# linto-ai/whisper-timestamped

Measured on NVIDIA H100. Metric: audio-sec/s (RTF) large-v3 1h synthetic @1/2/4/8 H100; DTW GB/s vs HBM peak, higher is better.
Workload: dtype bf16x3 tensor-core GEMMs (float32-accurate), f32 elsewhere, f64 DTW accumulate

## Files before the change

whisper-timestamped_b200/csrc/decode_steps.cu:

```cuda
#include "decode_common.cuh"

namespace wts {

constexpr int MG_THREADS = 256;
constexpr int MG_WARPS = MG_THREADS / 32;
constexpr int MG_MAXROWS = 32;
constexpr int MG_MAXNI = 10;

struct MgShared {
    int list[MG_MAXROWS];
    int n_active;
};

__device__ __forceinline__ float4 ldcg4(const float* p) { return __ldcg(reinterpret_cast<const float4*>(p)); }
__device__ __forceinline__ void prefetch_l2(const void* p) { asm volatile("prefetch.global.L2 [%0];" ::"l"(p)); }

enum { EPI_STORE = 0, EPI_ADD = 1, EPI_GELU = 2 };

__device__ __noinline__ void self_attention_task(const WtsDecodeSteps& P, const WtsDecLayer& Lr, int row, int h, int pos,
                                                    float* sc)
{
    const int lane = threadIdx.x & 31;
    const int D = P.D, n_ctx = P.n_ctx;
    float* Kc = Lr.self_k + ((int64_t)row * P.H + h) * n_ctx * 64;
    float* Vc = Lr.self_v + ((int64_t)row * P.H + h) * n_ctx * 64;
    const float* qrow = P.qkv + (int64_t)row * 3 * D + h * 64;
    {
        const float2 kn = __ldcg(reinterpret_cast<const float2*>(qrow + D) + lane);
        const float2 vn = __ldcg(reinterpret_cast<const float2*>(qrow + 2 * D) + lane);
        reinterpret_cast<float2*>(Kc + (int64_t)pos * 64)[lane] = kn;
        reinterpret_cast<float2*>(Vc + (int64_t)pos * 64)[lane] = vn;
        __threadfence_block();
        __syncwarp();
    }
    float q[64];
#pragma unroll
    for (int c = 0; c < 16; ++c) {
        const float4 t = ldcg4(qrow + 4 * c);
        q[4 * c] = t.x; q[4 * c + 1] = t.y; q[4 * c + 2] = t.z; q[4 * c + 3] = t.w;
    }
    const int nk = pos + 1;
    float mx = -CUDART_INF_F;
#pragma unroll 1
    for (int j = lane; j < nk; j += 32) {
        const float* kr = Kc + (int64_t)j * 64;
        float a = 0.f;
#pragma unroll
        for (int c = 0; c < 16; ++c) {
            const float4 kv = ldcg4(kr + 4 * c);
            a += q[4 * c] * kv.x + q[4 * c + 1] * kv.y + q[4 * c + 2] * kv.z + q[4 * c + 3] * kv.w;
        }
        sc[j] = a;
        mx = fmaxf(mx, a);
    }
    mx = warp_max(mx);
    float sum = 0.f;
#pragma unroll 1
    for (int j = lane; j < nk; j += 32) {
        const float e = expf(sc[j] - mx);
        sc[j] = e;
        sum += e;
    }
    sum = warp_sum(sum);
    __syncwarp();
    float2 o = make_float2(0.f, 0.f);
#pragma unroll 8
    for (int j = 0; j < nk; ++j) {
        const float p = sc[j];
        const float2 v = __ldcg(reinterpret_cast<const float2*>(Vc + (int64_t)j * 64) + lane);
        o.x = fmaf(p, v.x, o.x);
        o.y = fmaf(p, v.y, o.y);
    }
    const float inv = 1.0f / sum;
    reinterpret_cast<float2*>(P.att + (int64_t)row * D + h * 64)[lane] = make_float2(o.x * inv, o.y * inv);
    __syncwarp();
}

__device__ __noinline__ void cross_attention_phase(const WtsDecodeSteps& P, const WtsDecLayer& Lr, const MgShared& sh, float* xs)
{
    const int D = P.D, H = P.H;
    CaScratch& sc = *reinterpret_cast<CaScratch*>(xs);
    const int c8 = threadIdx.x & 7;
    for (int t = blockIdx.x; t < sh.n_active * H; t += gridDim.x) {
        const int row = sh.list[t / H], h = t % H;
        float qf[8];
        {
            const float* qp = P.q + (int64_t)row * D + h * 64 + c8 * 8;
            const float4 a = ldcg4(qp), b = ldcg4(qp + 4);
            qf[0] = a.x; qf[1] = a.y; qf[2] = a.z; qf[3] = a.w; qf[4] = b.x; qf[5] = b.y; qf[6] = b.z; qf[7] = b.w;
// ... 29 lines not shown
        }
        if (threadIdx.x == 0) sh.n_active = count <= MG_MAXROWS ? count : 0;
    }
    __syncthreads();
}

__global__ void __launch_bounds__(MG_THREADS)
lean_embed_kernel(const WtsDecodeSteps P)
{
    pdl_launch();
    pdl_wait();
    const int row = blockIdx.x;
    if (row >= P.cap || __ldcg(P.done + row) != 0) return;
    const int nt = __ldcg(P.n_tokens + row);
    const int tok = __ldcg(P.tokens + (int64_t)row * P.cfg.tokens_ld + nt - 1);
    const float* e = P.emb + (int64_t)tok * P.D;
    const float* p = P.pos + (int64_t)(nt - 1) * P.D;
    for (int c = threadIdx.x; c < P.D; c += MG_THREADS) P.x[(int64_t)row * P.D + c] = __ldg(e + c) + __ldg(p + c);
}

__global__ void __launch_bounds__(MG_THREADS)
lean_self_attn_kernel(const WtsDecodeSteps P, const WtsDecLayer* Lr)
{
    extern __shared__ __align__(16) unsigned char smem_raw[];
    MgShared& sh = *reinterpret_cast<MgShared*>(smem_raw);
    float* xs = reinterpret_cast<float*>(smem_raw + 1024);
    pdl_launch();
    pdl_wait();
    build_row_list(P, sh);
    const int warp = threadIdx.x >> 5;
    const int t = blockIdx.x * MG_WARPS + warp;
    if (t >= sh.n_active * P.H) return;
    const int row = sh.list[t / P.H];
    self_attention_task(P, *Lr, row, t % P.H, __ldcg(P.n_tokens + row) - 1, xs + warp * P.n_ctx);
}

__global__ void __launch_bounds__(MG_THREADS)
lean_cross_attn_kernel(const WtsDecodeSteps P, const WtsDecLayer* Lr)
{
    extern __shared__ __align__(16) unsigned char smem_raw[];
    MgShared& sh = *reinterpret_cast<MgShared*>(smem_raw);
    float* xs = reinterpret_cast<float*>(smem_raw + 1024);
    pdl_launch();
    pdl_wait();
    build_row_list(P, sh);
    if (blockIdx.x >= sh.n_active * P.H) return;
    cross_attention_phase(P, *Lr, sh, xs);
}

constexpr int LEAN_SELECT_THREADS = 1024;
__global__ void __launch_bounds__(LEAN_SELECT_THREADS)
lean_select_kernel(const WtsDecodeSteps P)
{
    __shared__ SelectScratch S;
    pdl_launch();
    pdl_wait();
    const int row = blockIdx.x;
    if (row >= P.cap || P.done[row] != 0) return;
    select_row(P.logits + (int64_t)row * P.cfg.n_vocab, P.cfg, P.suppress, P.blank, P.tokens + (int64_t)row * P.cfg.tokens_ld,
               P.n_tokens + row, P.n_prompt[row], P.done + row, P.logprobs + (int64_t)row * P.lp_ld,
               P.full != nullptr ? P.full + (int64_t)row * P.lp_ld * P.cfg.n_vocab : nullptr,
               P.last_full != nullptr ? P.last_full + (int64_t)row * P.cfg.n_vocab : nullptr, S);
}

__device__ __forceinline__ void mma_m16n8k16_bf16(float (&d)[4], uint32_t a0, uint32_t a1, uint32_t a2, uint32_t a3, uint32_t b0,
                                                  uint32_t b1)
{
    asm volatile("mma.sync.aligned.m16n8k16.row.col.f32.bf16.bf16.f32 {%0, %1, %2, %3}, {%4, %5, %6, %7}, {%8, %9}, {%0, %1, %2, %3};"
                 : "+f"(d[0]), "+f"(d[1]), "+f"(d[2]), "+f"(d[3]) : "r"(a0), "r"(a1), "r"(a2), "r"(a3), "r"(b0), "r"(b1));
}
__device__ __forceinline__ uint4 ldg_stream_u4(const void* p)
{
    uint4 v;
    asm volatile("ld.global.nc.L1::no_allocate.v4.u32 {%0, %1, %2, %3}, [%4];" : "=r"(v.x), "=r"(v.y), "=r"(v.z), "=r"(v.w) : "l"(p));
    return v;
}
__device__ __forceinline__ uint32_t pack_bf16x2(float lo_k, float hi_k)
{
    const __nv_bfloat162 v = __floats2bfloat162_rn(lo_k, hi_k);
    return *reinterpret_cast<const uint32_t*>(&v);
}

constexpr int MM_TASK_N = 8;

template <bool LN>
__device__ __forceinline__ void mma_stage(const float* src, int64_t ld, int col0, int kc, const float* __restrict__ gam,
                                          const float* __restrict__ bet, const MgShared& sh, uint32_t* Ah, uint32_t* Al, int pitchW)
{
    const int warp = threadIdx.x >> 5, lane = threadIdx.x & 31;
    const int NI = kc >> 7;
    for (int i = warp; i < sh.n_active; i += MG_WARPS) {
        const float* r = src + (int64_t)sh.list[i] * ld + col0;
        float4 v[MG_MAXNI];
#pragma unroll
        for (int k = 0; k < MG_MAXNI; ++k)
            if (k < NI) v[k] = ldcg4(r + 4 * (lane + 32 * k));
        if (LN) {
            float s = 0.f;
#pragma unroll
            for (int k = 0; k < MG_MAXNI; ++k)
                if (k < NI) s += (v[k].x + v[k].y) + (v[k].z + v[k].w);
            const float mean = warp_sum(s) / (float)kc;
            float q = 0.f;
#pragma unroll
            for (int k = 0; k < MG_MAXNI; ++k)
                if (k < NI) {
                    const float a = v[k].x - mean, b = v[k].y - mean, c = v[k].z - mean, d = v[k].w - mean;
                    q += (a * a + b * b) + (c * c + d * d);
                }
            const float rstd = 1.0f / sqrtf(warp_sum(q) / (float)kc + 1e-5f);
#pragma unroll
            for (int k = 0; k < MG_MAXNI; ++k)
                if (k < NI) {
                    const float4 g = __ldg(reinterpret_cast<const float4*>(gam) + lane + 32 * k);
                    const float4 b = __ldg(reinterpret_cast<const float4*>(bet) + lane + 32 * k);
                    v[k].x = (v[k].x - mean) * rstd * g.x + b.x;
                    v[k].y = (v[k].y - mean) * rstd * g.y + b.y;
                    v[k].z = (v[k].z - mean) * rstd * g.z + b.z;
                    v[k].w = (v[k].w - mean) * rstd * g.w + b.w;
                }
        }
#pragma unroll
        for (int k = 0; k < MG_MAXNI; ++k)
            if (k < NI) {
                const int f = lane + 32 * k;
                const int kb = f >> 3, j = f & 7;
                const int w0 = kb * 16 + ((j & 1) * 2) * 4 + (j >> 1);
                const float hx = __bfloat162float(__float2bfloat16_rn(v[k].x)), hy = __bfloat162float(__float2bfloat16_rn(v[k].y));
                const float hz = __bfloat162float(__float2bfloat16_rn(v[k].z)), hw = __bfloat162float(__float2bfloat16_rn(v[k].w));
                uint32_t* ah = Ah + (int64_t)i * pitchW;
                uint32_t* al = Al + (int64_t)i * pitchW;
                ah[w0] = pack_bf16x2(hx, hy);
                ah[w0 + 4] = pack_bf16x2(hz, hw);
                al[w0] = pack_bf16x2(v[k].x - hx, v[k].y - hy);
                al[w0 + 4] = pack_bf16x2(v[k].z - hz, v[k].w - hw);
            }
    }
}

template <int MT>
__global__ void __launch_bounds__(MG_THREADS, 1)
lean_mma_kernel(const WtsDecodeSteps P, const __nv_bfloat16* __restrict__ Whi, int64_t plane, int N, int K,
                const float* __restrict__ bias, const float* src, int64_t lds, const float* gam, const float* bet, float* out,
                int64_t ldo, int epi, int ln)
{
    extern __shared__ __align__(16) unsigned char smem_raw[];
    MgShared& sh = *reinterpret_cast<MgShared*>(smem_raw);
    const int D = P.D;
    const int KC = D;
    const int nchunks = K / KC;
    const int pitchW = (KC + 8) >> 1;
    uint32_t* Ah = reinterpret_cast<uint32_t*>(smem_raw + 1024);
    uint32_t* Al = Ah + (size_t)16 * MT * pitchW;
    float4* red = reinterpret_cast<float4*>(Al + (size_t)16 * MT * pitchW);
    const int warp = threadIdx.x >> 5, lane = threadIdx.x & 31;
    const int g = lane >> 2, q = lane & 3;
    const int ntasks = (N + MM_TASK_N - 1) / MM_TASK_N;
    pdl_launch();
    {
        const int lines_per_row = K / 64;
        for (int t = blockIdx.x, r = 0; t < ntasks && r < 2; t += gridDim.x, ++r)
            for (int ln_ = threadIdx.x; ln_ < MM_TASK_N * lines_per_row * 2; ln_ += MG_THREADS) {
                const int pl = ln_ / (MM_TASK_N * lines_per_row), rem = ln_ - pl * MM_TASK_N * lines_per_row;
                const int f = rem / lines_per_row, c = rem - f * lines_per_row;
                prefetch_l2(Whi + (int64_t)pl * plane + (int64_t)min(t * MM_TASK_N + f, N - 1) * K + c * 64);
            }
    }
    pdl_wait();
    build_row_list(P, sh);
    const int nA = sh.n_active;
    if (nA == 0) return;
    for (int idx = threadIdx.x; idx < (16 * MT - nA) * pitchW; idx += MG_THREADS) {
        Ah[(size_t)nA * pitchW + idx] = 0u;
        Al[(size_t)nA * pitchW + idx] = 0u;
    }
    const int nkb = KC >> 5;
    float acc[2][MT][4];
#pragma unroll
    for (int r = 0; r < 2; ++r)
#pragma unroll
        for (int m = 0; m < MT; ++m)
#pragma unroll
            for (int e = 0; e < 4; ++e) acc[r][m][e] = 0.f;

    auto task_partial = [&](int t, int c, float (&part)[MT][4]) {
        const int n = min(t * MM_TASK_N + g, N - 1);
        const __nv_bfloat16* wrow = Whi + (int64_t)n * K + (int64_t)c * KC + 8 * q;
#pragma unroll 1
        for (int kb0 = warp; kb0 < nkb; kb0 += 5 * MG_WARPS) {
            uint4 bh[5], bl[5];
#pragma unroll
            for (int u = 0; u < 5; ++u) {
                const int kb = kb0 + u * MG_WARPS;
                if (kb < nkb) {
                    bh[u] = ldg_stream_u4(wrow + kb * 32);
                    bl[u] = ldg_stream_u4(wrow + kb * 32 + plane);
                }
            }
#pragma unroll
            for (int u = 0; u < 5; ++u) {
                const int kb = kb0 + u * MG_WARPS;
                if (kb < nkb) {
#pragma unroll
                    for (int m = 0; m < MT; ++m) {
                        const uint32_t* ah0 = Ah + (size_t)(16 * m + g) * pitchW + kb * 16 + q;
                        const uint32_t* ah8 = ah0 + (size_t)8 * pitchW;
                        const uint32_t* al0 = Al + (size_t)(16 * m + g) * pitchW + kb * 16 + q;
                        const uint32_t* al8 = al0 + (size_t)8 * pitchW;
                        {
                            const uint32_t a0 = ah0[0], a1 = ah8[0], a2 = ah0[4], a3 = ah8[4];
                            const uint32_t l0 = al0[0], l1 = al8[0], l2 = al0[4], l3 = al8[4];
                            mma_m16n8k16_bf16(part[m], a0, a1, a2, a3, bh[u].x, bh[u].y);
                            mma_m16n8k16_bf16(part[m], l0, l1, l2, l3, bh[u].x, bh[u].y);
                            mma_m16n8k16_bf16(part[m], a0, a1, a2, a3, bl[u].x, bl[u].y);
                        }
                        {
                            const uint32_t a0 = ah0[8], a1 = ah8[8], a2 = ah0[12], a3 = ah8[12];
                            const uint32_t l0 = al0[8], l1 = al8[8], l2 = al0[12], l3 = al8[12];
                            mma_m16n8k16_bf16(part[m], a0, a1, a2, a3, bh[u].z, bh[u].w);
                            mma_m16n8k16_bf16(part[m], l0, l1, l2, l3, bh[u].z, bh[u].w);
                            mma_m16n8k16_bf16(part[m], a0, a1, a2, a3, bl[u].z, bl[u].w);
                        }
                    }
                }
            }
        }
    };
    auto task_finish = [&](int t, float (&part)[MT][4]) {
#pragma unroll
        for (int m = 0; m < MT; ++m) red[(warp * MT + m) * 32 + lane] = make_float4(part[m][0], part[m][1], part[m][2], part[m][3]);
        __syncthreads();
        if (warp < MT) {
            float4 s = red[(0 * MT + warp) * 32 + lane];
#pragma unroll
            for (int w = 1; w < MG_WARPS; ++w) {
                const float4 v = red[(w * MT + warp) * 32 + lane];
                s.x += v.x; s.y += v.y; s.z += v.z; s.w += v.w;
            }
            const float vals[4] = {s.x, s.y, s.z, s.w};
#pragma unroll
            for (int e = 0; e < 4; ++e) {
                const int ri = 16 * warp + g + ((e >> 1) ? 8 : 0);
                const int n = t * MM_TASK_N + 2 * q + (e & 1);
                if (ri < nA && n < N) {
                    float v = vals[e] + (bias != nullptr ? __ldg(bias + n) : 0.f);
                    float* dst = out + (int64_t)sh.list[ri] * ldo + n;
                    if (epi == EPI_GELU) v = gelu_erf(v);
                    else if (epi == EPI_ADD) v += __ldcg(dst);
                    *dst = v;
                }
            }
        }
        __syncthreads();
    };

    for (int c = 0; c < nchunks; ++c) {
        if (c > 0) __syncthreads();
        if (ln) mma_stage<true>(src, lds, c * KC, KC, gam, bet, sh, Ah, Al, pitchW);
        else    mma_stage<false>(src, lds, c * KC, KC, nullptr, nullptr, sh, Ah, Al, pitchW);
        __syncthreads();
        if (nchunks == 1) {
            for (int t = blockIdx.x; t < ntasks; t += gridDim.x) {
                float part[MT][4];
#pragma unroll
                for (int m = 0; m < MT; ++m)
#pragma unroll
                    for (int e = 0; e < 4; ++e) part[m][e] = 0.f;
                task_partial(t, 0, part);
                task_finish(t, part);
            }
        } else {
#pragma unroll
            for (int r = 0; r < 2; ++r) {
                const int t = blockIdx.x + r * gridDim.x;
                if (t < ntasks) task_partial(t, c, acc[r]);
            }
        }
    }
    if (nchunks > 1) {
#pragma unroll
        for (int r = 0; r < 2; ++r) {
            const int t = blockIdx.x + r * gridDim.x;
            if (t < ntasks) task_finish(t, acc[r]);
        }
    }
}

template <int MT>
static int launch_lean_step(const WtsDecodeSteps& P, const WtsDecLayer* h_layers, int n_sm, cudaStream_t st)
{
    const int D = P.D, H = P.H, V = P.cfg.n_vocab;
    const int pitchW = (D + 8) >> 1;
    const size_t sm_mma = 1024 + (size_t)2 * 16 * MT * pitchW * 4 + (size_t)MG_WARPS * MT * 32 * 16;
    const size_t sm_self = (size_t)MG_WARPS * P.n_ctx * sizeof(float) + 1024;
    const size_t sm_cross = sizeof(CaScratch) + 1024;
    static bool attr = false;
    if (!attr) {
        WTS_CUDA_CHECK(cudaFuncSetAttribute(lean_mma_kernel<MT>, cudaFuncAttributeMaxDynamicSharedMemorySize, 200 * 1024));
        attr = true;
    }
    if (sm_mma > 200 * 1024) { set_error("wts_decode_step_kernels: %zu bytes of shared memory needed", sm_mma); return -2; }
    const dim3 g_gemv(n_sm), blk(MG_THREADS);
    const dim3 g_self((P.max_rows * H + MG_WARPS - 1) / MG_WARPS), g_cross(P.max_rows * H);
    typedef const __nv_bfloat16* BF;
    const float* nof = nullptr;
    WTS_CUDA_CHECK(launch_pdl(lean_embed_kernel, dim3(P.cap), blk, 0, st, P));
    for (int li = 0; li < P.n_layer; ++li) {
        const WtsDecLayer& L = h_layers[li];
        const WtsDecLayer* dL = P.layers + li;
        WTS_CUDA_CHECK(launch_pdl(lean_mma_kernel<MT>, g_gemv, blk, sm_mma, st, P, (BF)L.sb_qkv, (int64_t)L.pl_qkv, 3 * D, D, L.b_qkv,
                                  (const float*)P.x, (int64_t)D, L.ln1_g, L.ln1_b, P.qkv, (int64_t)(3 * D), (int)EPI_STORE, 1));
        WTS_CUDA_CHECK(launch_pdl(lean_self_attn_kernel, g_self, blk, sm_self, st, P, dL));
        WTS_CUDA_CHECK(launch_pdl(lean_mma_kernel<MT>, g_gemv, blk, sm_mma, st, P, (BF)L.sb_o, (int64_t)L.pl_o, D, D, L.b_o,
                                  (const float*)P.att, (int64_t)D, nof, nof, P.x, (int64_t)D, (int)EPI_ADD, 0));
        WTS_CUDA_CHECK(launch_pdl(lean_mma_kernel<MT>, g_gemv, blk, sm_mma, st, P, (BF)L.sb_cq, (int64_t)L.pl_cq, D, D, L.b_cq,
                                  (const float*)P.x, (int64_t)D, L.ln2_g, L.ln2_b, P.q, (int64_t)D, (int)EPI_STORE, 1));
        WTS_CUDA_CHECK(launch_pdl(lean_cross_attn_kernel, g_cross, blk, sm_cross, st, P, dL));
        WTS_CUDA_CHECK(launch_pdl(lean_mma_kernel<MT>, g_gemv, blk, sm_mma, st, P, (BF)L.sb_co, (int64_t)L.pl_co, D, D, L.b_co,
                                  (const float*)P.att, (int64_t)D, nof, nof, P.x, (int64_t)D, (int)EPI_ADD, 0));
        WTS_CUDA_CHECK(launch_pdl(lean_mma_kernel<MT>, g_gemv, blk, sm_mma, st, P, (BF)L.sb_fc1, (int64_t)L.pl_fc1, 4 * D, D, L.b_fc1,
                                  (const float*)P.x, (int64_t)D, L.ln3_g, L.ln3_b, P.mid, (int64_t)(4 * D), (int)EPI_GELU, 1));
        WTS_CUDA_CHECK(launch_pdl(lean_mma_kernel<MT>, g_gemv, blk, sm_mma, st, P, (BF)L.sb_fc2, (int64_t)L.pl_fc2, D, 4 * D, L.b_fc2,
                                  (const float*)P.mid, (int64_t)(4 * D), nof, nof, P.x, (int64_t)D, (int)EPI_ADD, 0));
    }
    WTS_CUDA_CHECK(launch_pdl(lean_mma_kernel<MT>, g_gemv, blk, sm_mma, st, P, (BF)P.emb_sb, (int64_t)P.emb_plane, V, D, nof,
                              (const float*)P.x, (int64_t)D, P.ln_g, P.ln_b, P.logits, (int64_t)V, (int)EPI_STORE, 1));
    WTS_CUDA_CHECK(launch_pdl(lean_select_kernel, dim3(P.cap), dim3(LEAN_SELECT_THREADS), 0, st, P));
    return 0;
}

}

using namespace wts;

extern "C" int wts_decode_step_kernels(const WtsDecodeSteps* p, const WtsDecLayer* h_layers, void* stream)
{
    if (!p || !h_layers) { set_error("wts_decode_step_kernels: null argument"); return -2; }
    const WtsDecodeSteps& P = *p;
    if (P.D % 128 != 0 || P.D > 128 * MG_MAXNI || P.D != P.H * 64) {
        set_error("wts_decode_step_kernels: n_text_state %d not supported", P.D);
        return -2;
    }
    if (P.max_rows > MG_MAXROWS || P.max_rows < 1) { set_error("wts_decode_step_kernels: 1..%d active rows", MG_MAXROWS); return -2; }
    if ((size_t)MG_WARPS * P.n_ctx * sizeof(float) + 1024 > 48 * 1024) { set_error("wts_decode_step_kernels: n_text_ctx too large"); return -2; }
    if (P.emb_sb == nullptr) { set_error("wts_decode_step_kernels: no SB16 token embedding"); return -2; }
    static int n_sm = 0;
    if (n_sm == 0) {
        int dev = 0;
        WTS_CUDA_CHECK(cudaGetDevice(&dev));
        WTS_CUDA_CHECK(cudaDeviceGetAttribute(&n_sm, cudaDevAttrMultiProcessorCount, dev));
    }
    if (P.D / MM_TASK_N > 2 * n_sm) {
        set_error("wts_decode_step_kernels: n_text_state %d needs at least %d SMs, the device has %d", P.D, P.D / 16, n_sm);
        return -2;
    }
    cudaStream_t st = (cudaStream_t)stream;
    return P.max_rows <= 16 ? launch_lean_step<1>(P, h_layers, n_sm, st) : launch_lean_step<2>(P, h_layers, n_sm, st);
}
```

whisper-timestamped_b200/whisper_timestamped/engine.py:

```python
import ctypes
import os

import numpy as np
import torch

from . import _native as nat
from .alignment import attn_prep, dtw, plan_segments, split_jumps
from .model import SB16
from .windows import N_FRAMES, WindowRecord

N_SAMPLES = 480000
N_CTX_AUDIO = 1500
KPAD = 1504


def _i32(x, dev):
    return torch.as_tensor(np.asarray(x, dtype=np.int32)).to(dev)


class CudaEngine:
    def __init__(self, model, max_batch=None, gemm_backend=None, keep_full_logprobs=False, small_batch_rows=None):
        self.m = model
        self.dev = model.device
        self.w = model.w
        self.dims = model.dims
        self.max_batch = max_batch or int(os.environ.get("WTS_MAX_BATCH", "64"))
        self.backend = int(os.environ.get("WTS_GEMM_BACKEND", "0")) if gemm_backend is None else gemm_backend
        self.conv_backend = int(os.environ.get("WTS_CONV_BACKEND", str(self.backend)))
        self.fused_attention = os.environ.get("WTS_FUSED_ATTN", "1") != "0"
        self.keep_full_logprobs = keep_full_logprobs
        self.qk_buffers = []
        self.window_index = []
        self.full_logprobs = []
        self.launches = 0
        self.use_graph = os.environ.get("WTS_CUDA_GRAPH", "1") != "0"
        self.small_batch_rows = min(32, int(os.environ.get("WTS_SMALL_BATCH_ROWS", "8")) if small_batch_rows is None
                                    else int(small_batch_rows))
        self.small_batch_steps = 0
        self.decode_steps_run = 0
        self._graphs = {}
        self.profile = False
        self._events = []
        self.heads = None
        self.set_alignment_heads(model.heads)

    def set_alignment_heads(self, heads=None):
        heads = sorted((int(l), int(h)) for l, h in (self.m.heads if heads is None else heads))
        if heads == self.heads:
            return
        d = self.dims
        L, H = d.n_text_layer, d.n_text_head
        assert heads and all(0 <= l < L and 0 <= h < H for l, h in heads), heads
        assert len(set(heads)) == len(heads), "duplicate alignment heads"
        slots = torch.full((L, H), -1, dtype=torch.int32)
        for s_, (l, h) in enumerate(heads):
            slots[l, h] = s_
        self.heads = heads
        self.head_slot = slots.to(self.dev)
        counts = [sum(1 for l, _ in heads if l == li) for li in range(L)]
        self.layer_slots = [(sum(counts[:li]), counts[li]) for li in range(L)]
        self._session = None
        self._tf_state = None

    class _Phase:
        def __init__(self, eng, name):
            self.eng, self.name = eng, name

        def __enter__(self):
            if self.eng.profile:
                self.a = torch.cuda.Event(enable_timing=True)
                self.b = torch.cuda.Event(enable_timing=True)
                self.a.record(torch.cuda.current_stream(self.eng.dev))

        def __exit__(self, *exc):
            if self.eng.profile:
                self.b.record(torch.cuda.current_stream(self.eng.dev))
                self.eng._events.append((self.name, self.a, self.b))

    def phase(self, name):
        return CudaEngine._Phase(self, name)

    def stage_ms(self, reset=True):
        torch.cuda.synchronize(self.dev)
        out = {}
        self.batch_ms = [(B, steps, self._events[i][1].elapsed_time(self._events[i][2]))
                         for (B, steps, i) in getattr(self, "batch_log", [])]
        self.batch_log = []
        for name, a, b in self._events:
            out[name] = out.get(name, 0.0) + a.elapsed_time(b)
        if reset:
            self._events = []
        return out

    def _st(self):
        return nat.stream_ptr(self.dev)

    def gemm(self, a, b, M, N, K, *, lda=None, ldb=None, a_plane=None, b_plane=None, a_off=0, b_off=0,
             batch=(1, 1), a_b=(0, 0), b_b=(0, 0), alpha=1.0, bias=None, bias_on_m=False, act=0,
             residual=None, ldr=0, r_b=(0, 0), out_f32=None, ldc=0, c_b=(0, 0), c_off=0,
             out_sb=None, ldo=0, o_plane=0, o_b=(0, 0), o_off=0, head_dim=0, head_stride=0,
             a_f32=False, b_f32=False, backend=None, row_mask=None):
        g = nat.Gemm()
        if a_f32:
            g.a, g.lda, g.a_plane = a.data_ptr() + 4 * a_off, lda, 0
        else:
            g.a, g.lda, g.a_plane = a.ptr + 2 * a_off, lda or a.ld, a_plane if a_plane is not None else a.plane
        if b_f32:
            g.b, g.ldb, g.b_plane = b.data_ptr() + 4 * b_off, ldb, 0
        else:
            g.b, g.ldb, g.b_plane = b.ptr + 2 * b_off, ldb or b.ld, b_plane if b_plane is not None else b.plane
        g.a_bo, g.a_bi = a_b
        g.b_bo, g.b_bi = b_b
        g.M, g.N, g.K = M, N, K
        g.batch_outer, g.batch_inner = batch
        g.alpha = alpha
        g.bias = bias.data_ptr() if bias is not None else None
        g.bias_on_m = 1 if bias_on_m else 0
        g.act = act
        if residual is not None:
            g.residual, g.ldr = residual.data_ptr(), ldr
            g.r_bo, g.r_bi = r_b
        if out_f32 is not None:
            g.out_f32, g.ldc = out_f32.data_ptr() + 4 * c_off, ldc
            g.c_bo, g.c_bi = c_b
# ... 203 lines not shown
        limit = self.batch_limit(setup)
        for i in range(0, len(jobs), limit):
            out.extend(self._decode_batch(jobs[i:i + limit], setup))
        return out

    def window_bytes(self, sample_len):
        d = self.dims
        L, H, D, n_ctx = d.n_text_layer, d.n_text_head, d.n_text_state, d.n_text_ctx
        N, ctx = len(self.heads), N_CTX_AUDIO
        cross = L * H * ctx * 64 * 2 * 2 + N * ctx * 64 * 4 + H * ctx * 64 * 4
        self_kv = 2 * L * H * n_ctx * 64 * 4
        rows = 2 * N * (sample_len + 1) * ctx * 4
        Da = d.n_audio_state
        encoder = 3002 * d.n_mels * 4 + 3001 * Da * 4 + ctx * Da * (4 + 4 + 8 + 4 + 16 + 4) + Da * KPAD * 4
        return cross + self_kv + rows + encoder

    def batch_limit(self, setup):
        key = (tuple(self.heads), setup.sample_len)
        lim = getattr(self, "_limits", {})
        if key not in lim:
            torch.cuda.empty_cache()
            free, _ = torch.cuda.mem_get_info(self.dev)
            ses = getattr(self, "_session", None)
            if ses is not None:
                free += ses["cap"] * self.window_bytes(setup.sample_len)
            lim[key] = max(1, min(self.max_batch, int(0.85 * free) // self.window_bytes(setup.sample_len)))
            self._limits = lim
        return lim[key]

    def _decoder_session(self, setup, need):
        d, dev = self.dims, self.dev
        tok = setup.tokenizer
        V, D, n_ctx = d.n_vocab, d.n_text_state, d.n_text_ctx
        ses = getattr(self, "_session", None)
        cap = 4
        while cap < need:
            cap *= 2
        cap = min(cap, max(self.batch_limit(setup), need))
        if ses is not None and ses["cap"] >= need:
            cap = ses["cap"]
        key = (cap, setup.sample_len, tok.eot, tok.timestamp_begin, tok.no_timestamps, setup.max_initial_timestamp_index,
               self.keep_full_logprobs, self.small_batch_rows)
        if ses is not None and ses["key"] == key:
            return ses
        self._session = ses = None
        qk_rows = setup.sample_len + 1
        n_slots = len(self.heads)
        i32 = dict(dtype=torch.int32, device=dev)
        ses = dict(key=key, cap=cap, qk_rows=qk_rows, graph=None, per_step=0)
        ses["st8"] = self._alloc_decoder_state(cap, cap)
        ses["st8"]["hs_fin"] = SB16(cap, D, dev)
        ses["tokens"] = torch.zeros((cap, n_ctx + 1), **i32)
        ses["n_tokens"] = torch.ones(cap, **i32)
        ses["n_prompt"] = torch.ones(cap, **i32)
        ses["done"] = torch.ones(cap, **i32)
        ses["logprobs"] = torch.zeros((cap, qk_rows), dtype=torch.float32, device=dev)
        ses["full"] = torch.empty((cap, qk_rows, V), dtype=torch.float32, device=dev) if self.keep_full_logprobs else None
        ses["qk_buf"] = torch.zeros((cap, max(1, n_slots), qk_rows, N_CTX_AUDIO), dtype=torch.float32, device=dev)
        ses["qk_out"] = torch.zeros_like(ses["qk_buf"])
        ses["qk_out_idx"] = None
        ses["s_tok"] = torch.zeros(cap, **i32)
        ses["s_pos"] = torch.zeros(cap, **i32)
        ses["s_qkr"] = torch.zeros(cap, **i32)
        ses["s_act"] = torch.zeros(cap, **i32)
        ses["seq_ids"] = _i32(list(range(cap)), dev)
        ses["logits"] = torch.empty((cap, V), dtype=torch.float32, device=dev)
        ses["xs"] = torch.empty((cap, D), dtype=torch.float32, device=dev)
        ses["last_full"] = torch.zeros((cap, V), dtype=torch.float32, device=dev)
        ses["suppress"] = torch.zeros(V, dtype=torch.uint8, device=dev)
        ses["blank"] = torch.zeros(V, dtype=torch.uint8, device=dev)
        ses["cfg"] = nat.DecodeCfg(n_vocab=V, eot=tok.eot, timestamp_begin=tok.timestamp_begin,
                                   no_timestamps=tok.no_timestamps,
                                   max_initial_ts=-1 if setup.max_initial_timestamp_index is None else setup.max_initial_timestamp_index,
                                   sample_len=setup.sample_len, n_ctx=n_ctx, tokens_ld=n_ctx + 1)
        ses["steps"] = self._steps_descriptor(ses) if self.small_batch_rows > 0 else None
        self._session = ses
        return ses

    def _steps_descriptor(self, ses):
        d, w, dev = self.dims, self.w, self.dev
        D, H, L, V = d.n_text_state, d.n_text_head, d.n_text_layer, d.n_vocab
        if D % 128 != 0 or D > 1280 or D != 64 * H:
            return None
        if D // 8 > 2 * torch.cuda.get_device_properties(dev).multi_processor_count:
            return None
        st8, cap = ses["st8"], ses["cap"]
        layers = (nat.DecLayer * L)()
        for li, blk in enumerate(w.dec):
            a, c, y = blk.attn, blk.cross, layers[li]
            y.ln1_g, y.ln1_b, y.b_qkv, y.b_o = a.ln_g.data_ptr(), a.ln_b.data_ptr(), a.qkv_b.data_ptr(), a.out_b.data_ptr()
            y.ln2_g, y.ln2_b, y.b_cq, y.b_co = c.ln_g.data_ptr(), c.ln_b.data_ptr(), c.q_b.data_ptr(), c.out_b.data_ptr()
            y.ln3_g, y.ln3_b = blk.mlp_ln_g.data_ptr(), blk.mlp_ln_b.data_ptr()
            y.b_fc1, y.b_fc2 = blk.fc1_b.data_ptr(), blk.fc2_b.data_ptr()
            y.self_k, y.self_v = st8["sk"][li].data_ptr(), st8["sv"][li].data_ptr()
            y.cross_k16, y.cross_v16 = st8["ck"][li].data_ptr(), st8["cv"][li].data_ptr()
            kal = st8["ckal"][li]
            y.cross_k_align, y.head_slot = kal.data_ptr() if kal is not None else None, self.head_slot[li].data_ptr()
            y.align_s0, y.align_n = self.layer_slots[li]
            for name, sb in (("qkv", a.qkv), ("o", a.out), ("cq", c.q), ("co", c.out), ("fc1", blk.fc1), ("fc2", blk.fc2)):
                assert sb.ld == sb.cols
                setattr(y, "sb_" + name, sb.ptr)
                setattr(y, "pl_" + name, sb.plane)
        raw = np.frombuffer(bytes(layers), dtype=np.uint8).copy()
        f32 = dict(dtype=torch.float32, device=dev)
        keep = dict(layers=torch.from_numpy(raw).to(dev), x=torch.zeros((cap, D), **f32), qkv=torch.zeros((cap, 3 * D), **f32),
                    att=torch.zeros((cap, D), **f32), q=torch.zeros((cap, D), **f32), mid=torch.zeros((cap, 4 * D), **f32))
        p = nat.DecodeSteps()
        p.layers = keep["layers"].data_ptr()
        p.emb, p.pos, p.ln_g, p.ln_b = w.emb.data_ptr(), w.dec_pos.data_ptr(), w.ln_g.data_ptr(), w.ln_b.data_ptr()
        p.tokens, p.n_tokens, p.n_prompt, p.done = (ses[k].data_ptr() for k in ("tokens", "n_tokens", "n_prompt", "done"))
        p.logprobs, p.qk_buf = ses["logprobs"].data_ptr(), ses["qk_buf"].data_ptr()
        p.full = ses["full"].data_ptr() if ses["full"] is not None else None
        p.last_full = ses["last_full"].data_ptr()
        p.suppress, p.blank = ses["suppress"].data_ptr(), ses["blank"].data_ptr()
        p.x, p.qkv, p.att, p.q, p.mid = (keep[k].data_ptr() for k in ("x", "qkv", "att", "q", "mid"))
        p.logits = ses["logits"].data_ptr()
        p.emb_sb, p.emb_plane = w.emb_sb.ptr, w.emb_sb.plane
        p.cfg = ses["cfg"]
        p.n_layer, p.D, p.H, p.n_ctx, p.n_audio_ctx = L, D, H, d.n_text_ctx, N_CTX_AUDIO
        p.n_slots, p.cap, p.lp_ld, p.qk_rows = len(self.heads), cap, ses["qk_rows"], ses["qk_rows"]
        return dict(args=p, keep=keep, host_layers=layers, graphs={})

    def _capture(self, ses, run):
        dev = self.dev
        saved = {k: ses[k].clone() for k in ("tokens", "n_tokens", "done", "logprobs")}
        run()
        torch.cuda.synchronize(dev)
        for k, v in saved.items():
            ses[k].copy_(v)
        graph = torch.cuda.CUDAGraph()
        cap_stream = torch.cuda.Stream(device=dev)
        cap_stream.wait_stream(torch.cuda.current_stream(dev))
        with torch.cuda.stream(cap_stream):
            with torch.cuda.graph(graph, stream=cap_stream):
                run()
        torch.cuda.current_stream(dev).wait_stream(cap_stream)
        return graph

    def _lean_graph(self, ses, n_active):
        sd = ses["steps"]
        rows = 4 if n_active <= 4 else 8 if n_active <= 8 else 16 if n_active <= 16 else 32
        if rows not in sd["graphs"]:
            p = sd["args"]

            def launch():
                p.max_rows = rows
                nat.check(nat.lib.wts_decode_step_kernels(ctypes.byref(p), ctypes.byref(sd["host_layers"]), self._st()),
                          "wts_decode_step_kernels")
            sd["graphs"][rows] = self._capture(ses, launch)
        return sd["graphs"][rows]

    def _step_graph(self, ses):
        if ses["graph"] is None:
            l0 = self.launches
            ses["graph"] = self._capture(ses, lambda: self._step(ses))
            ses["per_step"] = (self.launches - l0) // 2
            self.launches -= ses["per_step"]
        return ses["graph"]

    def _decode_chunk(self, ses, n_active, chunk, max_steps):
        if ses["steps"] is not None and n_active <= self.small_batch_rows:
            graph = self._lean_graph(ses, n_active)
            for _ in range(chunk):
                graph.replay()
            self.launches += chunk * (8 * self.dims.n_text_layer + 3)
            self.small_batch_steps += chunk
        else:
            graph = self._step_graph(ses) if (self.use_graph and max_steps > 4) else None
            for _ in range(chunk):
                if graph is not None:
                    graph.replay()
                    self.launches += ses["per_step"]
                else:
                    self._step(ses)
        self.decode_steps_run += chunk

    def _set_masks(self, ses, setup):
        dev = self.dev
        ses["suppress"].zero_()
        ses["suppress"][torch.as_tensor(list(setup.suppress_tokens), dtype=torch.long, device=dev)] = 1
        ses["blank"].zero_()
        if setup.blank_tokens:
            ses["blank"][torch.as_tensor(list(setup.blank_tokens), dtype=torch.long, device=dev)] = 1

    def _prefill(self, ses, prompts, slots, tok, qk_last):
        d, dev, st, w = self.dims, self.dev, self._st(), self.w
        D, V = d.n_text_state, d.n_vocab
        n = len(prompts)
        P = [len(p) for p in prompts]
        R0 = sum(P)
        row_seq = _i32([b for b, p in zip(slots, prompts) for _ in p], dev)
        row_pos = _i32([i for p in prompts for i in range(len(p))], dev)
        row_tok = _i32([t for p in prompts for t in p], dev)
        qk_row = _i32([0 if qk_last and i == len(p) - 1 else -1 for p in prompts for i in range(len(p))], dev)
        f32 = dict(dtype=torch.float32, device=dev)
        pre = dict(ses["st8"])
        pre.update(hs=SB16(R0, D, dev), att=SB16(R0, D, dev), mid=SB16(R0, 4 * D, dev),
                   qkv=torch.empty((R0, 3 * D), **f32), q=torch.empty((R0, D), **f32))
        x = torch.empty((R0, D), **f32)
        nat.check(nat.lib.wts_embed(row_tok.data_ptr(), row_pos.data_ptr(), w.emb.data_ptr(), w.dec_pos.data_ptr(), R0, D,
                                    x.data_ptr(), st), "wts_embed")
        self._decoder_rows(pre, x, R0, row_seq, row_pos, qk_row, ses["qk_buf"])
        ends = np.cumsum(P) - 1
        sot_rows = [int(ends[k] - P[k] + 1 + prompts[k].index(tok.sot)) for k in range(n)]
        sel = _i32(list(ends) + sot_rows, dev)
        xr = torch.empty((2 * n, D), **f32)
        nat.check(nat.lib.wts_gather_rows(x.data_ptr(), D, sel.data_ptr(), 2 * n, D, xr.data_ptr(), st), "wts_gather_rows")
        logits2 = torch.empty((2 * n, V), **f32)
        self._final_logits(xr, 2 * n, logits2)
        no_speech = torch.zeros(n, **f32)
        if tok.no_speech is not None:
            nat.check(nat.lib.wts_softmax_pick(logits2.data_ptr() + 4 * n * V, V, V, tok.no_speech, no_speech.data_ptr(), n, st),
                      "wts_softmax_pick")
        return logits2, no_speech

    def _select(self, ses, logits, rows):
        d = self.dims
        nat.check(nat.lib.wts_decode_select(logits.data_ptr(), d.n_vocab, ctypes.byref(ses["cfg"]), ses["suppress"].data_ptr(),
                                            ses["blank"].data_ptr(), ses["tokens"].data_ptr(), ses["n_tokens"].data_ptr(),
                                            ses["n_prompt"].data_ptr(), ses["done"].data_ptr(), ses["logprobs"].data_ptr(),
                                            ses["qk_rows"], ses["full"].data_ptr() if ses["full"] is not None else None,
                                            ses["last_full"].data_ptr(), rows, self._st()), "wts_decode_select")
        self.launches += 1

    def _step(self, ses):
        self._step_logits(ses)
        self._select(ses, ses["logits"], ses["cap"])
        self.launches += 1

    def _step_logits(self, ses):
        d, w, st = self.dims, self.w, self._st()
        cap, D = ses["cap"], d.n_text_state
        nat.check(nat.lib.wts_step_inputs(ses["tokens"].data_ptr(), d.n_text_ctx + 1, ses["n_tokens"].data_ptr(),
                                          ses["n_prompt"].data_ptr(), ses["done"].data_ptr(), cap, ses["s_tok"].data_ptr(),
                                          ses["s_pos"].data_ptr(), ses["s_qkr"].data_ptr(), ses["s_act"].data_ptr(), st),
                  "wts_step_inputs")
        nat.check(nat.lib.wts_embed(ses["s_tok"].data_ptr(), ses["s_pos"].data_ptr(), w.emb.data_ptr(), w.dec_pos.data_ptr(),
                                    cap, D, ses["xs"].data_ptr(), st), "wts_embed")
        self._decoder_rows(ses["st8"], ses["xs"], cap, ses["seq_ids"], ses["s_pos"], ses["s_qkr"], ses["qk_buf"],
                           active=ses["s_act"])
        self._final_logits_static(ses["xs"], cap, ses["logits"], ses["st8"], active=ses["s_act"])
        self.launches += 1

    @torch.no_grad()
# ... 465 lines not shown
```

Measured before the change: 524.7.

## Split lean decode GEMV rows across CTA pairs and double-buffer weight loads

Extends the lean small-batch decode path from 32 to 64 active rows. When more than 32 rows are active, it splits rows across pairs of CTAs, each covering a 32-row slice, and lets each CTA handle up to three N-tasks. The weight loads are restructured into a job loop that double-buffers register fragments, so the next job's weights are fetched while the current job's MMAs run. This raises register pressure and halves the task-parallel grid when the split is used. Whether the new row range is used at all depends on WTS_SMALL_BATCH_ROWS, which defaults to 8.

Result: no change. 523.9, median of 6 (-0.1%).

```diff
diff --git a/whisper-timestamped_b200/csrc/decode_steps.cu b/whisper-timestamped_b200/csrc/decode_steps.cu
--- a/whisper-timestamped_b200/csrc/decode_steps.cu
+++ b/whisper-timestamped_b200/csrc/decode_steps.cu
@@ -4,7 +4,8 @@
 
 constexpr int MG_THREADS = 256;
 constexpr int MG_WARPS = MG_THREADS / 32;
-constexpr int MG_MAXROWS = 32;
+constexpr int MG_MAXROWS = 64;
+constexpr int MG_CTA_ROWS = 32;
 constexpr int MG_MAXNI = 10;
 
 struct MgShared {
@@ -200,15 +201,17 @@
 }
 
 constexpr int MM_TASK_N = 8;
+constexpr int MM_MAX_TASKS = 3;
 
 template <bool LN>
 __device__ __forceinline__ void mma_stage(const float* src, int64_t ld, int col0, int kc, const float* __restrict__ gam,
-                                          const float* __restrict__ bet, const MgShared& sh, uint32_t* Ah, uint32_t* Al, int pitchW)
+                                          const float* __restrict__ bet, const int* rows, int nrows, uint32_t* Ah, uint32_t* Al,
+                                          int pitchW)
 {
     const int warp = threadIdx.x >> 5, lane = threadIdx.x & 31;
     const int NI = kc >> 7;
-    for (int i = warp; i < sh.n_active; i += MG_WARPS) {
-        const float* r = src + (int64_t)sh.list[i] * ld + col0;
+    for (int i = warp; i < nrows; i += MG_WARPS) {
+        const float* r = src + (int64_t)rows[i] * ld + col0;
         float4 v[MG_MAXNI];
 #pragma unroll
         for (int k = 0; k < MG_MAXNI; ++k)
@@ -260,7 +263,7 @@
 __global__ void __launch_bounds__(MG_THREADS, 1)
 lean_mma_kernel(const WtsDecodeSteps P, const __nv_bfloat16* __restrict__ Whi, int64_t plane, int N, int K,
                 const float* __restrict__ bias, const float* src, int64_t lds, const float* gam, const float* bet, float* out,
-                int64_t ldo, int epi, int ln)
+                int64_t ldo, int epi, int ln, int nsplit)
 {
     extern __shared__ __align__(16) unsigned char smem_raw[];
     MgShared& sh = *reinterpret_cast<MgShared*>(smem_raw);
@@ -274,10 +277,30 @@
     const int warp = threadIdx.x >> 5, lane = threadIdx.x & 31;
     const int g = lane >> 2, q = lane & 3;
     const int ntasks = (N + MM_TASK_N - 1) / MM_TASK_N;
+    const int t0 = blockIdx.x / nsplit, tstep = gridDim.x / nsplit;
+    const int my_tasks = t0 < ntasks ? (ntasks - 1 - t0) / tstep + 1 : 0;
+    const int nkb = KC >> 5;
+    const int njobs = my_tasks * nchunks;
+    auto load_w = [&](int j, uint4 (&bh)[5], uint4 (&bl)[5]) {
+        const int c = j / my_tasks, t = t0 + (j - c * my_tasks) * tstep;
+        const int n = min(t * MM_TASK_N + g, N - 1);
+        const __nv_bfloat16* wrow = Whi + (int64_t)n * K + (int64_t)c * KC + 8 * q;
+#pragma unroll
+        for (int u = 0; u < 5; ++u) {
+            const int kb = warp + u * MG_WARPS;
+            bh[u] = bl[u] = make_uint4(0u, 0u, 0u, 0u);
+            if (kb < nkb) {
+                bh[u] = ldg_stream_u4(wrow + kb * 32);
+                bl[u] = ldg_stream_u4(wrow + kb * 32 + plane);
+            }
+        }
+    };
+    uint4 wh0[5], wl0[5], wh1[5], wl1[5];
     pdl_launch();
+    if (njobs > 0) load_w(0, wh0, wl0);
     {
         const int lines_per_row = K / 64;
-        for (int t = blockIdx.x, r = 0; t < ntasks && r < 2; t += gridDim.x, ++r)
+        for (int t = t0 + tstep, r = 0; t < ntasks && r < 2; t += tstep, ++r)
             for (int ln_ = threadIdx.x; ln_ < MM_TASK_N * lines_per_row * 2; ln_ += MG_THREADS) {
                 const int pl = ln_ / (MM_TASK_N * lines_per_row), rem = ln_ - pl * MM_TASK_N * lines_per_row;
                 const int f = rem / lines_per_row, c = rem - f * lines_per_row;
@@ -286,59 +309,46 @@
     }
     pdl_wait();
     build_row_list(P, sh);
-    const int nA = sh.n_active;
-    if (nA == 0) return;
+    const int r0 = (blockIdx.x % nsplit) * MG_CTA_ROWS;
+    const int nA = min(sh.n_active - r0, 16 * MT);
+    if (nA <= 0) return;
+    const int* rows = sh.list + r0;
     for (int idx = threadIdx.x; idx < (16 * MT - nA) * pitchW; idx += MG_THREADS) {
         Ah[(size_t)nA * pitchW + idx] = 0u;
         Al[(size_t)nA * pitchW + idx] = 0u;
     }
-    const int nkb = KC >> 5;
-    float acc[2][MT][4];
-#pragma unroll
-    for (int r = 0; r < 2; ++r)
+    float acc[MM_MAX_TASKS][MT][4];
+#pragma unroll
+    for (int r = 0; r < MM_MAX_TASKS; ++r)
 #pragma unroll
         for (int m = 0; m < MT; ++m)
 #pragma unroll
             for (int e = 0; e < 4; ++e) acc[r][m][e] = 0.f;
 
-    auto task_partial = [&](int t, int c, float (&part)[MT][4]) {
-        const int n = min(t * MM_TASK_N + g, N - 1);
-        const __nv_bfloat16* wrow = Whi + (int64_t)n * K + (int64_t)c * KC + 8 * q;
-#pragma unroll 1
-        for (int kb0 = warp; kb0 < nkb; kb0 += 5 * MG_WARPS) {
-            uint4 bh[5], bl[5];
-#pragma unroll
-            for (int u = 0; u < 5; ++u) {
-                const int kb = kb0 + u * MG_WARPS;
-                if (kb < nkb) {
-                    bh[u] = ldg_stream_u4(wrow + kb * 32);
-                    bl[u] = ldg_stream_u4(wrow + kb * 32 + plane);
-                }
-            }
-#pragma unroll
-            for (int u = 0; u < 5; ++u) {
-                const int kb = kb0 + u * MG_WARPS;
-                if (kb < nkb) {
-#pragma unroll
-                    for (int m = 0; m < MT; ++m) {
-                        const uint32_t* ah0 = Ah + (size_t)(16 * m + g) * pitchW + kb * 16 + q;
-                        const uint32_t* ah8 = ah0 + (size_t)8 * pitchW;
-                        const uint32_t* al0 = Al + (size_t)(16 * m + g) * pitchW + kb * 16 + q;
-                        const uint32_t* al8 = al0 + (size_t)8 * pitchW;
-                        {
-                            const uint32_t a0 = ah0[0], a1 = ah8[0], a2 = ah0[4], a3 = ah8[4];
-                            const uint32_t l0 = al0[0], l1 = al8[0], l2 = al0[4], l3 = al8[4];
-                            mma_m16n8k16_bf16(part[m], a0, a1, a2, a3, bh[u].x, bh[u].y);
-                            mma_m16n8k16_bf16(part[m], l0, l1, l2, l3, bh[u].x, bh[u].y);
-                            mma_m16n8k16_bf16(part[m], a0, a1, a2, a3, bl[u].x, bl[u].y);
-                        }
-                        {
-                            const uint32_t a0 = ah0[8], a1 = ah8[8], a2 = ah0[12], a3 = ah8[12];
-                            const uint32_t l0 = al0[8], l1 = al8[8], l2 = al0[12], l3 = al8[12];
-                            mma_m16n8k16_bf16(part[m], a0, a1, a2, a3, bh[u].z, bh[u].w);
-                            mma_m16n8k16_bf16(part[m], l0, l1, l2, l3, bh[u].z, bh[u].w);
-                            mma_m16n8k16_bf16(part[m], a0, a1, a2, a3, bl[u].z, bl[u].w);
-                        }
+    auto mma_w = [&](const uint4 (&bh)[5], const uint4 (&bl)[5], float (&part)[MT][4]) {
+#pragma unroll
+        for (int u = 0; u < 5; ++u) {
+            const int kb = warp + u * MG_WARPS;
+            if (kb < nkb) {
+#pragma unroll
+                for (int m = 0; m < MT; ++m) {
+                    const uint32_t* ah0 = Ah + (size_t)(16 * m + g) * pitchW + kb * 16 + q;
+                    const uint32_t* ah8 = ah0 + (size_t)8 * pitchW;
+                    const uint32_t* al0 = Al + (size_t)(16 * m + g) * pitchW + kb * 16 + q;
+                    const uint32_t* al8 = al0 + (size_t)8 * pitchW;
+                    {
+                        const uint32_t a0 = ah0[0], a1 = ah8[0], a2 = ah0[4], a3 = ah8[4];
+                        const uint32_t l0 = al0[0], l1 = al8[0], l2 = al0[4], l3 = al8[4];
+                        mma_m16n8k16_bf16(part[m], a0, a1, a2, a3, bh[u].x, bh[u].y);
+                        mma_m16n8k16_bf16(part[m], l0, l1, l2, l3, bh[u].x, bh[u].y);
+                        mma_m16n8k16_bf16(part[m], a0, a1, a2, a3, bl[u].x, bl[u].y);
+                    }
+                    {
+                        const uint32_t a0 = ah0[8], a1 = ah8[8], a2 = ah0[12], a3 = ah8[12];
+                        const uint32_t l0 = al0[8], l1 = al8[8], l2 = al0[12], l3 = al8[12];
+                        mma_m16n8k16_bf16(part[m], a0, a1, a2, a3, bh[u].z, bh[u].w);
+                        mma_m16n8k16_bf16(part[m], l0, l1, l2, l3, bh[u].z, bh[u].w);
+                        mma_m16n8k16_bf16(part[m], a0, a1, a2, a3, bl[u].z, bl[u].w);
                     }
                 }
             }
@@ -362,7 +372,7 @@
                 const int n = t * MM_TASK_N + 2 * q + (e & 1);
                 if (ri < nA && n < N) {
                     float v = vals[e] + (bias != nullptr ? __ldg(bias + n) : 0.f);
-                    float* dst = out + (int64_t)sh.list[ri] * ldo + n;
+                    float* dst = out + (int64_t)rows[ri] * ldo + n;
                     if (epi == EPI_GELU) v = gelu_erf(v);
                     else if (epi == EPI_ADD) v += __ldcg(dst);
                     *dst = v;
@@ -371,38 +381,43 @@
         }
         __syncthreads();
     };
-
-    for (int c = 0; c < nchunks; ++c) {
-        if (c > 0) __syncthreads();
-        if (ln) mma_stage<true>(src, lds, c * KC, KC, gam, bet, sh, Ah, Al, pitchW);
-        else    mma_stage<false>(src, lds, c * KC, KC, nullptr, nullptr, sh, Ah, Al, pitchW);
-        __syncthreads();
+    auto run_job = [&](int j, const uint4 (&bh)[5], const uint4 (&bl)[5]) {
+        const int c = j / my_tasks, r = j - c * my_tasks;
+        if (r == 0) {
+            if (c > 0) __syncthreads();
+            if (ln) mma_stage<true>(src, lds, c * KC, KC, gam, bet, rows, nA, Ah, Al, pitchW);
+            else    mma_stage<false>(src, lds, c * KC, KC, nullptr, nullptr, rows, nA, Ah, Al, pitchW);
+            __syncthreads();
+        }
         if (nchunks == 1) {
-            for (int t = blockIdx.x; t < ntasks; t += gridDim.x) {
-                float part[MT][4];
-#pragma unroll
-                for (int m = 0; m < MT; ++m)
-#pragma unroll
-                    for (int e = 0; e < 4; ++e) part[m][e] = 0.f;
-                task_partial(t, 0, part);
-                task_finish(t, part);
-            }
+            float part[MT][4];
+#pragma unroll
+            for (int m = 0; m < MT; ++m)
+#pragma unroll
+                for (int e = 0; e < 4; ++e) part[m][e] = 0.f;
+            mma_w(bh, bl, part);
+            task_finish(t0 + r * tstep, part);
         } else {
 #pragma unroll
-            for (int r = 0; r < 2; ++r) {
-                const int t = blockIdx.x + r * gridDim.x;
-                if (t < ntasks) task_partial(t, c, acc[r]);
-            }
-        }
+            for (int rr = 0; rr < MM_MAX_TASKS; ++rr)
+                if (rr == r) mma_w(bh, bl, acc[rr]);
+        }
+    };
+    for (int j = 0; j < njobs; j += 2) {
+        if (j + 1 < njobs) load_w(j + 1, wh1, wl1);
+        run_job(j, wh0, wl0);
+        if (j + 1 >= njobs) break;
+        if (j + 2 < njobs) load_w(j + 2, wh0, wl0);
+        run_job(j + 1, wh1, wl1);
     }
     if (nchunks > 1) {
 #pragma unroll
-        for (int r = 0; r < 2; ++r) {
-            const int t = blockIdx.x + r * gridDim.x;
-            if (t < ntasks) task_finish(t, acc[r]);
-        }
-    }
-}
+        for (int r = 0; r < MM_MAX_TASKS; ++r)
+            if (r < my_tasks) task_finish(t0 + r * tstep, acc[r]);
+    }
+}
+
+static int lean_nsplit(int max_rows) { return max_rows > MG_CTA_ROWS ? 2 : 1; }
 
 template <int MT>
 static int launch_lean_step(const WtsDecodeSteps& P, const WtsDecLayer* h_layers, int n_sm, cudaStream_t st)
@@ -418,7 +433,8 @@
         attr = true;
     }
     if (sm_mma > 200 * 1024) { set_error("wts_decode_step_kernels: %zu bytes of shared memory needed", sm_mma); return -2; }
-    const dim3 g_gemv(n_sm), blk(MG_THREADS);
+    const int nsplit = lean_nsplit(P.max_rows);
+    const dim3 g_gemv(n_sm / nsplit * nsplit), blk(MG_THREADS);
     const dim3 g_self((P.max_rows * H + MG_WARPS - 1) / MG_WARPS), g_cross(P.max_rows * H);
     typedef const __nv_bfloat16* BF;
     const float* nof = nullptr;
@@ -427,22 +443,22 @@
         const WtsDecLayer& L = h_layers[li];
         const WtsDecLayer* dL = P.layers + li;
         WTS_CUDA_CHECK(launch_pdl(lean_mma_kernel<MT>, g_gemv, blk, sm_mma, st, P, (BF)L.sb_qkv, (int64_t)L.pl_qkv, 3 * D, D, L.b_qkv,
-                                  (const float*)P.x, (int64_t)D, L.ln1_g, L.ln1_b, P.qkv, (int64_t)(3 * D), (int)EPI_STORE, 1));
+                                  (const float*)P.x, (int64_t)D, L.ln1_g, L.ln1_b, P.qkv, (int64_t)(3 * D), (int)EPI_STORE, 1, nsplit));
         WTS_CUDA_CHECK(launch_pdl(lean_self_attn_kernel, g_self, blk, sm_self, st, P, dL));
         WTS_CUDA_CHECK(launch_pdl(lean_mma_kernel<MT>, g_gemv, blk, sm_mma, st, P, (BF)L.sb_o, (int64_t)L.pl_o, D, D, L.b_o,
-                                  (const float*)P.att, (int64_t)D, nof, nof, P.x, (int64_t)D, (int)EPI_ADD, 0));
+                                  (const float*)P.att, (int64_t)D, nof, nof, P.x, (int64_t)D, (int)EPI_ADD, 0, nsplit));
         WTS_CUDA_CHECK(launch_pdl(lean_mma_kernel<MT>, g_gemv, blk, sm_mma, st, P, (BF)L.sb_cq, (int64_t)L.pl_cq, D, D, L.b_cq,
-                                  (const float*)P.x, (int64_t)D, L.ln2_g, L.ln2_b, P.q, (int64_t)D, (int)EPI_STORE, 1));
+                                  (const float*)P.x, (int64_t)D, L.ln2_g, L.ln2_b, P.q, (int64_t)D, (int)EPI_STORE, 1, nsplit));
         WTS_CUDA_CHECK(launch_pdl(lean_cross_attn_kernel, g_cross, blk, sm_cross, st, P, dL));
         WTS_CUDA_CHECK(launch_pdl(lean_mma_kernel<MT>, g_gemv, blk, sm_mma, st, P, (BF)L.sb_co, (int64_t)L.pl_co, D, D, L.b_co,
-                                  (const float*)P.att, (int64_t)D, nof, nof, P.x, (int64_t)D, (int)EPI_ADD, 0));
+                                  (const float*)P.att, (int64_t)D, nof, nof, P.x, (int64_t)D, (int)EPI_ADD, 0, nsplit));
         WTS_CUDA_CHECK(launch_pdl(lean_mma_kernel<MT>, g_gemv, blk, sm_mma, st, P, (BF)L.sb_fc1, (int64_t)L.pl_fc1, 4 * D, D, L.b_fc1,
-                                  (const float*)P.x, (int64_t)D, L.ln3_g, L.ln3_b, P.mid, (int64_t)(4 * D), (int)EPI_GELU, 1));
+                                  (const float*)P.x, (int64_t)D, L.ln3_g, L.ln3_b, P.mid, (int64_t)(4 * D), (int)EPI_GELU, 1, nsplit));
         WTS_CUDA_CHECK(launch_pdl(lean_mma_kernel<MT>, g_gemv, blk, sm_mma, st, P, (BF)L.sb_fc2, (int64_t)L.pl_fc2, D, 4 * D, L.b_fc2,
-                                  (const float*)P.mid, (int64_t)(4 * D), nof, nof, P.x, (int64_t)D, (int)EPI_ADD, 0));
+                                  (const float*)P.mid, (int64_t)(4 * D), nof, nof, P.x, (int64_t)D, (int)EPI_ADD, 0, nsplit));
     }
     WTS_CUDA_CHECK(launch_pdl(lean_mma_kernel<MT>, g_gemv, blk, sm_mma, st, P, (BF)P.emb_sb, (int64_t)P.emb_plane, V, D, nof,
-                              (const float*)P.x, (int64_t)D, P.ln_g, P.ln_b, P.logits, (int64_t)V, (int)EPI_STORE, 1));
+                              (const float*)P.x, (int64_t)D, P.ln_g, P.ln_b, P.logits, (int64_t)V, (int)EPI_STORE, 1, nsplit));
     WTS_CUDA_CHECK(launch_pdl(lean_select_kernel, dim3(P.cap), dim3(LEAN_SELECT_THREADS), 0, st, P));
     return 0;
 }
@@ -468,8 +484,10 @@
         WTS_CUDA_CHECK(cudaGetDevice(&dev));
         WTS_CUDA_CHECK(cudaDeviceGetAttribute(&n_sm, cudaDevAttrMultiProcessorCount, dev));
     }
-    if (P.D / MM_TASK_N > 2 * n_sm) {
-        set_error("wts_decode_step_kernels: n_text_state %d needs at least %d SMs, the device has %d", P.D, P.D / 16, n_sm);
+    const int nsplit = lean_nsplit(P.max_rows);
+    if (P.D / MM_TASK_N > MM_MAX_TASKS * (n_sm / nsplit)) {
+        set_error("wts_decode_step_kernels: n_text_state %d at %d active rows needs at least %d SMs, the device has %d", P.D,
+                  P.max_rows, nsplit * ((P.D / MM_TASK_N + MM_MAX_TASKS - 1) / MM_MAX_TASKS), n_sm);
         return -2;
     }
     cudaStream_t st = (cudaStream_t)stream;
diff --git a/whisper-timestamped_b200/whisper_timestamped/engine.py b/whisper-timestamped_b200/whisper_timestamped/engine.py
--- a/whisper-timestamped_b200/whisper_timestamped/engine.py
+++ b/whisper-timestamped_b200/whisper_timestamped/engine.py
@@ -16,6 +16,10 @@
 
 def _i32(x, dev):
     return torch.as_tensor(np.asarray(x, dtype=np.int32)).to(dev)
+
+
+LEAN_MAX_ROWS = 64
+LEAN_GRID_ROWS = (4, 8, 16, 32, 48, 64)
 
 
 class CudaEngine:
@@ -34,12 +38,13 @@
         self.full_logprobs = []
         self.launches = 0
         self.use_graph = os.environ.get("WTS_CUDA_GRAPH", "1") != "0"
-        self.small_batch_rows = min(32, int(os.environ.get("WTS_SMALL_BATCH_ROWS", "8")) if small_batch_rows is None
-                                    else int(small_batch_rows))
+        self.small_batch_rows = min(LEAN_MAX_ROWS, int(os.environ.get("WTS_SMALL_BATCH_ROWS", "8"))
+                                    if small_batch_rows is None else int(small_batch_rows))
         self.small_batch_steps = 0
         self.decode_steps_run = 0
         self._graphs = {}
         self.profile = False
+        self.row_log = []
         self._events = []
         self.heads = None
         self.set_alignment_heads(model.heads)
@@ -409,8 +414,10 @@
         D, H, L, V = d.n_text_state, d.n_text_head, d.n_text_layer, d.n_vocab
         if D % 128 != 0 or D > 1280 or D != 64 * H:
             return None
-        if D // 8 > 2 * torch.cuda.get_device_properties(dev).multi_processor_count:
+        n_sm = torch.cuda.get_device_properties(dev).multi_processor_count
+        if D // 8 > 3 * n_sm:
             return None
+        max_rows = LEAN_MAX_ROWS if D // 8 <= 3 * (n_sm // 2) else 32
         st8, cap = ses["st8"], ses["cap"]
         layers = (nat.DecLayer * L)()
         for li, blk in enumerate(w.dec):
@@ -446,7 +453,7 @@
         p.cfg = ses["cfg"]
         p.n_layer, p.D, p.H, p.n_ctx, p.n_audio_ctx = L, D, H, d.n_text_ctx, N_CTX_AUDIO
         p.n_slots, p.cap, p.lp_ld, p.qk_rows = len(self.heads), cap, ses["qk_rows"], ses["qk_rows"]
-        return dict(args=p, keep=keep, host_layers=layers, graphs={})
+        return dict(args=p, keep=keep, host_layers=layers, graphs={}, max_rows=max_rows)
 
     def _capture(self, ses, run):
         dev = self.dev
@@ -466,7 +473,8 @@
 
     def _lean_graph(self, ses, n_active):
         sd = ses["steps"]
-        rows = 4 if n_active <= 4 else 8 if n_active <= 8 else 16 if n_active <= 16 else 32
+        assert n_active <= sd["max_rows"], (n_active, sd["max_rows"])
+        rows = next(r for r in LEAN_GRID_ROWS if n_active <= r)
         if rows not in sd["graphs"]:
             p = sd["args"]
 
@@ -486,7 +494,9 @@
         return ses["graph"]
 
     def _decode_chunk(self, ses, n_active, chunk, max_steps):
-        if ses["steps"] is not None and n_active <= self.small_batch_rows:
+        if self.profile:
+            self.row_log.append((n_active, chunk))
+        if ses["steps"] is not None and n_active <= min(self.small_batch_rows, ses["steps"]["max_rows"]):
             graph = self._lean_graph(ses, n_active)
             for _ in range(chunk):
                 graph.replay()
```
